# V2AI/EFG

Hardware: AMD Instinct MI355X
Metric: scenes/sec ConQueR 1-frame Waymo train step (higher is better)
Workload: dtype f32; 1 GPU; ConQueR res18 p3, 1-sweep Waymo-shaped scenes, 180000 pts/scene, 0.1 m voxels, 2 scenes/GPU, 900 queries, fwd+bwd+AdamW+OneCycle, graph of `value`: FPN levels / heads the reference evaluates and never reads are skipped (same losses and gradients; the line's `full_graph` object times the full reference graph); global_batch=2, parallelism=dp1

## Files before the change

efg_amd/_lib.py:

```python
import ctypes
import os

import torch

_LIB_PATH = os.path.join(os.path.dirname(os.path.abspath(__file__)), "lib", "libefg_hip.so")
_lib = None

c_void_p, c_int, c_int64, c_size_t, c_float = (ctypes.c_void_p, ctypes.c_int, ctypes.c_int64, ctypes.c_size_t,
                                               ctypes.c_float)

_SIGS = {
    "efg_last_error": (ctypes.c_char_p, []),
    "efg_version": (ctypes.c_char_p, []),
    "efg_capture_stream_create": (ctypes.c_int, [ctypes.POINTER(ctypes.c_void_p)]),
    "efg_capture_stream_destroy": (ctypes.c_int, [ctypes.c_void_p]),
    "efg_dynamic_voxelize_f32": (c_int, [c_void_p, c_int64, c_int, c_void_p, c_void_p, c_void_p, c_void_p]),
    "efg_hard_voxelize_workspace_bytes": (c_size_t, [c_int64, c_int, c_int, c_int, c_int, c_void_p, c_void_p]),
    "efg_hard_voxelize_f32": (c_int, [c_void_p, c_void_p, c_int, c_int, c_void_p, c_void_p, c_int, c_int, c_void_p,
                                      c_void_p, c_int, c_void_p, c_void_p, c_void_p, c_void_p, c_size_t, c_void_p]),
    "efg_hard_voxelize_debug_timeline": (c_size_t, [c_void_p]),
    "efg_scatter_workspace_bytes": (c_size_t, [c_int64, c_int, c_void_p]),
    "efg_scatter_index": (c_int, [c_void_p, c_int64, c_int, c_void_p, c_void_p, c_void_p, c_void_p, c_size_t,
                                  c_void_p]),
    "efg_scatter_reduce_workspace_bytes": (c_size_t, [c_int64, c_int]),
# ... 70 lines not shown
    "efg_focal_loss_forward_f32": (c_int, [c_void_p, c_void_p, c_int, c_int64, c_int, c_float, c_float, c_void_p, c_void_p,
                                           c_void_p]),
    "efg_focal_loss_backward_f32": (c_int, [c_void_p, c_void_p, c_int, c_int64, c_int, c_float, c_float, c_void_p,
                                            c_void_p, c_void_p, c_void_p]),
    "efg_box_loss_forward_f32": (c_int, [c_void_p] * 6 + [c_int64] + [c_int] * 4 + [c_void_p] * 3),
    "efg_box_loss_backward_f32": (c_int, [c_void_p] * 6 + [c_int64] + [c_int] * 4 + [c_void_p] * 4),
    "efg_rot_giou_paired_forward_f32": (c_int, [c_void_p, c_void_p, c_int64] + [c_void_p] * 4),
    "efg_rot_giou_paired_backward_f32": (c_int, [c_void_p, c_void_p, c_int64] + [c_void_p] * 5),
    "efg_match_cost_rot_f32": (c_int, [c_void_p] * 4 + [c_int] * 5 + [c_float] * 6 + [c_void_p] * 3),
    "efg_box_loss_rot_forward_f32": (c_int, [c_void_p] * 6 + [c_int64] + [c_int] * 4 + [c_void_p] * 4),
    "efg_box_loss_rot_backward_f32": (c_int, [c_void_p] * 6 + [c_int64] + [c_int] * 4 + [c_void_p] * 5),
    "efg_bn_workspace_bytes": (c_size_t, [c_int]),
    "efg_bn_forward_f32": (c_int, [c_void_p] * 7 + [c_float, c_float, c_int64, c_int, c_int] + [c_void_p] * 4 +
                           [c_size_t, c_void_p]),
    "efg_bn_backward_f32": (c_int, [c_void_p] * 6 + [c_int64, c_int, c_int] + [c_void_p] * 5 + [c_size_t, c_void_p]),
    "efg_lsap_f32": (c_int, [c_void_p, c_int, c_int, c_int, c_void_p, c_void_p, c_void_p, c_void_p]),
    "efg_nms_f32": (c_int, [c_void_p, c_int, c_float, c_int, c_void_p, c_void_p, c_void_p, c_size_t, c_void_p]),
    "efg_spconv_tile_shape": (c_int, [c_int, c_int, c_int, c_int64, c_int64, c_void_p, c_void_p, c_void_p]),
    "efg_cylinder_select_f32": (c_int, [c_void_p, c_int64, c_int, c_int, c_float, c_void_p, c_void_p, c_int64, c_void_p,
                                        c_void_p, c_void_p, c_int, c_void_p, c_void_p]),
    "efg_attention_fwd_f32": (c_int, [c_void_p, c_int64, c_int64, c_void_p, c_void_p, c_int64, c_int64, c_int64, c_int, c_int,
                                      c_int, c_float, c_void_p, c_void_p, c_void_p]),
    "efg_attention_bwd_f32": (c_int, [c_void_p, c_int64, c_int64, c_void_p, c_void_p, c_int64, c_int64, c_void_p, c_void_p,
                                      c_void_p, c_int64, c_int, c_int, c_int, c_float, c_void_p, c_void_p, c_void_p,
                                      c_void_p]),
    "efg_attention_long_fwd_f32": (c_int, [c_void_p, c_int64, c_int64] * 3 + [c_void_p, c_int, c_int64, c_int, c_int, c_float,
                                                                             c_void_p, c_void_p, c_void_p]),
    "efg_attention_long_bwd_f32": (c_int, [c_void_p, c_int64, c_int64] * 3 + [c_void_p, c_int, c_void_p, c_void_p, c_void_p,
                                                                             c_int64, c_int, c_int, c_float, c_void_p, c_void_p,
                                                                             c_void_p, c_void_p, c_void_p]),
# ... 107 lines not shown
```

efg_amd/csrc/batchnorm.hip:

```cpp
#include "common.h"

#include <algorithm>

namespace efg {
namespace {

constexpr int kBnBlocks = 1024;

__device__ __forceinline__ float4 ld4(const float* p) { return *reinterpret_cast<const float4*>(p); }
__device__ __forceinline__ void st4(float* p, float4 v) { *reinterpret_cast<float4*>(p) = v; }

struct Chunk {
  long long row_lo, row_hi;
};
__device__ __forceinline__ Chunk chunk_of(long long m, int nblocks, int b) {
  const long long per = (m + nblocks - 1) / nblocks;
  Chunk c;
  c.row_lo = min((long long)b * per, m);
  c.row_hi = min(c.row_lo + per, m);
  return c;
}

__device__ __forceinline__ float4 quad_sum(float4 v, int q4, float4* smem) {
  smem[threadIdx.x] = v;
// ... 206 lines not shown
    d.y = yy.y > 0.f ? d.y : 0.f;
    d.z = yy.z > 0.f ? d.z : 0.f;
    d.w = yy.w > 0.f ? d.w : 0.f;
  }
  if (dres) st4(dres + e * 4, d);
  const float4 mu = ld4(mean + ch), is = ld4(invstd + ch), ww = ld4(w + ch), a1 = ld4(dbias + ch), a2 = ld4(dweight + ch);
  const float inv_m = 1.0f / (float)m;
  float4 o;
  o.x = (d.x - a1.x * inv_m - (v.x - mu.x) * is.x * a2.x * inv_m) * is.x * ww.x;
  o.y = (d.y - a1.y * inv_m - (v.y - mu.y) * is.y * a2.y * inv_m) * is.y * ww.y;
  o.z = (d.z - a1.z * inv_m - (v.z - mu.z) * is.z * a2.z * inv_m) * is.z * ww.z;
  o.w = (d.w - a1.w * inv_m - (v.w - mu.w) * is.w * a2.w * inv_m) * is.w * ww.w;
  st4(dx + e * 4, o);
}


__global__ void __launch_bounds__(64)
gn_stats_merge_kernel(const float* __restrict__ partial, int nchunks, int c, int cpg, float eps,
                      float* __restrict__ mean_out, float* __restrict__ rstd_out) {
  const int lane = threadIdx.x, g = blockIdx.x, b = blockIdx.y, groups = c / cpg;
  const float* base = partial + (long long)b * nchunks * 3 * c;
  float cnt = 0.f, mean = 0.f, M2 = 0.f;
  const int items = nchunks * cpg;
  for (int i0 = lane; i0 < items; i0 += 64 * 8) {
    float nbv[8], mbv[8], qbv[8];
#pragma unroll
    for (int u = 0; u < 8; ++u) {
      const int i = min(i0 + 64 * u, items - 1);
      const float* p = base + (long long)(i / cpg) * 3 * c + g * cpg + i % cpg;
      nbv[u] = (i0 + 64 * u < items) ? p[0] : 0.f;
// ... 184 lines not shown
                "batch_norm backward: null pointer");
  EFG_CHECK_ARG(ws_bytes >= efg_bn_workspace_bytes(c), "batch_norm backward: workspace too small");
  hipStream_t st = (hipStream_t)stream;
  const int nb = nblocks_for(m);
  hipLaunchKernelGGL(bn_bwd_reduce_kernel, dim3(nb), dim3(256), 0, st, dy, x, y, mean, invstd, (long long)m, c, relu,
                     static_cast<float*>(ws));
  hipLaunchKernelGGL(bn_bwd_merge_kernel, dim3(2 * c), dim3(64), 0, st, static_cast<const float*>(ws), nb, c, dbias, dweight);
  EFG_LAUNCH_CHECK();
  const long long total4 = (long long)m * c / 4;
  hipLaunchKernelGGL(bn_bwd_apply_kernel, dim3((unsigned)ceil_div(total4, 256)), dim3(256), 0, st, dy, x, y, weight, mean,
                     invstd, dbias, dweight, total4, (long long)m, c, relu, dx, dresidual);
  EFG_LAUNCH_CHECK();
  return EFG_OK;
}

extern "C" size_t efg_gn_workspace_bytes(int batch, int c) {
  if (batch < 1 || c < 1) return 0;
  return align_up(sizeof(float) * ((size_t)batch * kBnBlocks * 3 * c + (size_t)batch * 4 * c), 256) + 256;
}

static int gn_check(int batch, int64_t rows, int c, int groups) {
  EFG_CHECK_ARG(batch >= 1 && batch <= 65535 && rows >= 1, "group_norm: need batch in [1, 65535] and rows >= 1");
  EFG_CHECK_ARG(c >= 4 && c % 4 == 0 && c <= 1024, "group_norm: need c %% 4 == 0 and c <= 1024 (got %d)", c);
  EFG_CHECK_ARG(groups >= 1 && c % groups == 0 && (c / groups) % 4 == 0,
                "group_norm: channels per group must be a multiple of 4 (c = %d, groups = %d)", c, groups);
  return EFG_OK;
}

extern "C" int efg_gn_forward_f32(const float* x, const float* weight, const float* bias, float eps, int batch,
                                  int64_t rows, int c, int groups, float* y, float* mean, float* rstd, void* ws,
// ... 40 lines not shown
```

efg_amd/modeling/backbones/fpn.py:

```python
import math

import torch.nn.functional as F
from torch import nn

from ..common import Conv2d, c2_xavier_fill, get_norm
from .sparse_net import ShapeSpec, _get, build_sparse_resnet_backbone


class LastLevelMaxPool(nn.Module):

    def __init__(self, in_feature="p5"):
        super().__init__()
        self.num_levels = 1
        self.in_feature = in_feature

    def forward(self, x):
        return [F.max_pool2d(x, kernel_size=1, stride=2, padding=0)]


class FPN(nn.Module):
    def __init__(self, bottom_up, in_features, out_channels, norm="", top_block=None, fuse_type="sum"):
        super().__init__()
        self.out_channels = out_channels
        input_shapes = bottom_up.output_shape()
# ... 35 lines not shown
    @property
    def size_divisibility(self):
        return self._size_divisibility

    def set_active_levels(self, levels):
        self.active_levels = None if levels is None else list(levels)
        if levels is None:
            self.bottom_up.dense_features = None
            return
        lvl_names = ["p{}".format(int(math.log2(s))) for s in
                     [self.bottom_up.output_shape()[f].stride for f in self.in_features]]
        need = [n in levels for n in lvl_names]
        first = min(i for i, n in enumerate(need) if n)
        self.bottom_up.dense_features = self.in_features[first:]

    def forward(self, *args, **kwargs):
        bottom_up_features = self.bottom_up(*args, **kwargs)
        self.__dict__["last_bottom_up"] = bottom_up_features
        levels = ["p{}".format(int(math.log2(self._out_feature_strides[n]))) for n in self._out_features]
        active = set(levels) if self.active_levels is None else set(self.active_levels)
        names_td = [n for n in self._out_features if n in
                    {"p{}".format(int(math.log2(self.bottom_up.output_shape()[f].stride))) for f in self.in_features}]
        names_td = names_td[::-1]
        feats = self.in_features[::-1]
        results = {}
        prev = None
        for name, f, lateral_conv, output_conv in zip(names_td, feats, self.lateral_convs, self.output_convs):
            finer_needed = any(n in active for n in names_td[names_td.index(name):])
            if not finer_needed:
                break
            lat = lateral_conv(bottom_up_features[f])
            if prev is not None:
                lat = lat + F.interpolate(prev, scale_factor=2, mode="nearest")
                if self._fuse_type == "avg":
                    lat = lat / 2
            prev = lat
            if name in active:
                results[name] = output_conv(prev)
        if self.top_block is not None:
            top_names = [n for n in self._out_features if n not in names_td]
            if any(n in active for n in top_names):
                src = bottom_up_features.get(self.top_block.in_feature, None)
                if src is None:
                    if self.top_block.in_feature not in results:
                        i = names_td.index(self.top_block.in_feature)
                        raise RuntimeError("top block input %s was not evaluated" % names_td[i])
                    src = results[self.top_block.in_feature]
                for n, r in zip(top_names, self.top_block(src)):
                    results[n] = r
        return {n: results[n] for n in self._out_features if n in results}

    def output_shape(self):
        return {name: ShapeSpec(channels=self._out_feature_channels[name], stride=self._out_feature_strides[name])
# ... 10 lines not shown
```

efg_amd/modeling/common/__init__.py:

```python
import os

import torch
import torch.nn.functional as F
from torch import nn

from ...operators import batchnorm as _bn
from ...operators import linear as _linear_mod
from ...operators.conv2d import arm_covers, conv3x3, conv3x3_arm, deterministic_mode
from ...operators.linear import linear


def get_norm(norm, out_channels):
    args = None
    if isinstance(norm, (list, tuple)):
        norm, args = norm
    if isinstance(norm, str):
        if len(norm) == 0:
            return None
        norm = {
            "BN": nn.BatchNorm2d,
            "BN1d": nn.BatchNorm1d,
            "GN": lambda channels: nn.GroupNorm(32, channels),
            "nnSyncBN": nn.SyncBatchNorm,
        }[norm]
# ... 7 lines not shown
    inplace = activation["inplace"] if isinstance(activation, dict) else activation.inplace
    return {"ReLU": nn.ReLU, "ReLU6": nn.ReLU6}[atype](inplace=inplace)


class Conv2d(nn.Conv2d):

    def __init__(self, *args, norm=None, activation=None, **kwargs):
        super().__init__(*args, **kwargs)
        self.norm = norm
        self.activation = activation

    def _is_pointwise(self):
        return (self.kernel_size == (1, 1) and self.stride == (1, 1) and self.padding == (0, 0)
                and self.dilation == (1, 1) and self.groups == 1)

    def forward(self, x):
        if self._is_pointwise():
            y = linear(x.permute(0, 2, 3, 1), self.weight.view(self.out_channels, self.in_channels), self.bias)
            x = y.permute(0, 3, 1, 2)
        elif (x.is_cuda and self.kernel_size == (3, 3) and self.stride == (1, 1) and self.padding == (1, 1)
              and self.dilation == (1, 1) and self.groups == 1 and torch.is_grad_enabled() and deterministic_mode()):
            x = conv3x3(x, self.weight, self.bias)
        elif (x.is_cuda and self.kernel_size == (3, 3) and self.stride == (1, 1) and self.padding == (1, 1)
              and self.dilation == (1, 1) and self.groups == 1 and torch.is_grad_enabled()
              and _linear_mod.arm_active() is not None
              and os.environ.get("EFG_CONV2D_ARM", "1") != "0" and arm_covers(x, self.weight)):
            x = conv3x3_arm(x, self.weight, self.bias)
        else:
            x = super().forward(x)
        if self.norm is not None:
            if _bn.fusable_nhwc(self.norm, x):
                relu = type(self.activation) is nn.ReLU
                x = _bn.bn_act_nhwc(x, self.norm, relu)
                if relu:
# ... 13 lines not shown
```

efg_amd/operators/batchnorm.py:

```python
import os

import torch
from torch.autograd import Function
from torch.autograd.function import once_differentiable

from .. import _lib as L

class BatchNormActFunction(Function):
    @staticmethod
    def forward(ctx, x, residual, weight, bias, running_mean, running_var, num_batches_tracked, momentum, eps, relu):
        x = x.contiguous()
        m, c = x.shape
        res = residual.contiguous() if residual is not None else None
        y = torch.empty_like(x)
        mean = torch.empty(c, dtype=torch.float32, device=x.device)
        invstd = torch.empty(c, dtype=torch.float32, device=x.device)
        ws_bytes = L.lib().efg_bn_workspace_bytes(c)
        ws = torch.empty(ws_bytes, dtype=torch.uint8, device=x.device)
        L.check(L.lib().efg_bn_forward_f32(L.ptr(x), L.ptr(res), L.ptr(weight), L.ptr(bias), L.ptr(running_mean),
                                           L.ptr(running_var), L.ptr(num_batches_tracked), float(momentum), float(eps),
                                           m, c, 1 if relu else 0, L.ptr(y), L.ptr(mean), L.ptr(invstd), L.ptr(ws),
                                           ws_bytes, L.stream()))
        ctx.save_for_backward(x, y, weight, mean, invstd)
        ctx.relu, ctx.has_residual = bool(relu), residual is not None
# ... 4 lines not shown
    @once_differentiable
    def backward(ctx, dy):
        x, y, weight, mean, invstd = ctx.saved_tensors
        m, c = x.shape
        dy = dy.contiguous()
        dx = torch.empty_like(x)
        dres = torch.empty_like(x) if ctx.has_residual else None
        dweight = torch.empty(c, dtype=torch.float32, device=x.device)
        dbias = torch.empty(c, dtype=torch.float32, device=x.device)
        ws_bytes = L.lib().efg_bn_workspace_bytes(c)
        ws = torch.empty(ws_bytes, dtype=torch.uint8, device=x.device)
        L.check(L.lib().efg_bn_backward_f32(L.ptr(dy), L.ptr(x), L.ptr(y), L.ptr(weight), L.ptr(mean), L.ptr(invstd), m,
                                            c, 1 if ctx.relu else 0, L.ptr(dx), L.ptr(dres), L.ptr(dweight),
                                            L.ptr(dbias), L.ptr(ws), ws_bytes, L.stream()))
        return dx, dres, dweight, dbias, None, None, None, None, None, None


def fusable(bn, x):
    return (os.environ.get("EFG_FUSED_BN", "1") != "0" and isinstance(bn, torch.nn.BatchNorm1d) and bn.training
            and bn.affine and bn.track_running_stats and bn.momentum is not None and x.is_cuda
            and x.dtype == torch.float32 and x.dim() == 2 and x.shape[0] >= 2 and x.shape[1] % 4 == 0
            and x.shape[1] <= 1024)


def bn_act(x, bn, relu=False, residual=None):
    if not fusable(bn, x):
        y = bn(x)
        if residual is not None:
            y = y + residual
        return torch.relu(y) if relu else y
# ... 33 lines not shown
```

efg_amd/operators/conv2d.py:

```python
import os

import torch
import torch.nn.functional as F
from torch.autograd import Function
from torch.autograd.function import once_differentiable

from .linear import arm_module, weight_grad


def deterministic_mode():
    return os.environ.get("EFG_DETERMINISTIC", "0") == "1"


def _pad_rows(t, front):
    b, c, h, w = t.shape
    r = b * (h + 2) * (w + 2)
    rows = (r + 15) // 16 * 16
    buf = torch.zeros((front + rows + front, c), dtype=t.dtype, device=t.device)
    buf[front:front + r].view(b, h + 2, w + 2, c)[:, 1:-1, 1:-1].copy_(t.permute(0, 2, 3, 1))
    return buf, r, rows


def _unpad_rows(flat, b, h, w):
    return flat[:b * (h + 2) * (w + 2)].view(b, h + 2, w + 2, -1)[:, 1:-1, 1:-1].permute(0, 3, 1, 2)


_TAPS = [(ky, kx) for ky in range(3) for kx in range(3)]


def _taps_gemm(buf, rows, front, wp, mats, sign, bias=None):
    out = (bias.expand(rows, -1).contiguous() if bias is not None else
           torch.zeros((rows, mats[0].shape[1]), dtype=buf.dtype, device=buf.device))
    for (ky, kx), m in zip(_TAPS, mats):
        s = front + sign * ((ky - 1) * wp + (kx - 1))
        out.addmm_(buf[s:s + rows], m)
    return out


def wgrad_3x3(x, gy, xb=None):
    b, ci, h, w = gy.shape[0], (x.shape[1] if xb is None else xb.shape[1]), gy.shape[2], gy.shape[3]
    co = gy.shape[1]
    wp = w + 2
    front = wp + 1
    if xb is None:
        xb, _, _ = _pad_rows(x, front)
    gb, _, rows = _pad_rows(gy, 0)
    parts = []
    for ky, kx in _TAPS:
        s = front + (ky - 1) * wp + (kx - 1)
        parts.append(weight_grad(xb[s:s + rows], gb))
    return torch.stack(parts, dim=-1).view(co, ci, 3, 3)


class Conv3x3Function(Function):
    @staticmethod
    def forward(ctx, x, weight, bias):
        b, _, h, w = x.shape
        front = w + 3
        xb, _, rows = _pad_rows(x, front)
        ctx.save_for_backward(xb, weight)
        ctx.has_bias = bias is not None
        ctx.geom = (b, h, w)
        mats = [weight[:, :, ky, kx].t() for ky, kx in _TAPS]
        return _unpad_rows(_taps_gemm(xb, rows, front, w + 2, mats, +1, bias), b, h, w)

    @staticmethod
    @once_differentiable
    def backward(ctx, gy):
        xb, weight = ctx.saved_tensors
        b, h, w = ctx.geom
        front = w + 3
        gx = gw = gb = None
        if ctx.needs_input_grad[0]:
            gbuf, _, rows = _pad_rows(gy, front)
            mats = [weight[:, :, ky, kx] for ky, kx in _TAPS]
            gx = _unpad_rows(_taps_gemm(gbuf, rows, front, w + 2, mats, -1), b, h, w)
        if ctx.needs_input_grad[1]:
            gw = wgrad_3x3(None, gy, xb=xb).contiguous(memory_format=torch.channels_last if weight.is_contiguous(
                memory_format=torch.channels_last) and not weight.is_contiguous() else torch.contiguous_format)
        if ctx.has_bias and ctx.needs_input_grad[2]:
            gb = gy.sum((0, 2, 3))
        return gx, gw, gb


def conv3x3(x, weight, bias):
    return Conv3x3Function.apply(x, weight, bias)


def _tap_rows(buf, start_row, rows, c):
    return buf.as_strided((rows, 3 * c), (c, 1), buf.storage_offset() + start_row * c)


def _arm_products():
    return arm_module(default="bf16x3")
# ... 61 lines not shown
```

include/efg_hip.h:

```cpp
#ifndef EFG_HIP_H
#define EFG_HIP_H
#include <stddef.h>
#include <stdint.h>

#ifdef __cplusplus
extern "C" {
#endif

#define EFG_OK 0
#define EFG_E_INVALID (-1)
#define EFG_E_WORKSPACE (-2)
#define EFG_E_HIP (-3)

const char* efg_last_error(void);
const char* efg_version(void);

int efg_capture_stream_create(void** stream_out);
int efg_capture_stream_destroy(void* stream);


int efg_dynamic_voxelize_f32(const float* points, int64_t n, int f, const float* voxel_size_host,
                             const float* coors_range_host, int32_t* coors, void* stream);

size_t efg_hard_voxelize_workspace_bytes(int64_t n_total, int batch, int f, int max_points, int max_voxels,
// ... 209 lines not shown
int efg_topk_unsorted_f32(const float* x, int64_t rows, int n, int k, float* values, int64_t* indices, void* stream);

int efg_box_refine_forward_f32(const float* delta, const float* anchor, int64_t n, float eps, float* out, void* stream);
int efg_box_refine_backward_f32(const float* grad, const float* out, const float* anchor, int64_t n, float eps,
                                float* grad_delta, float* grad_anchor, void* stream);

size_t efg_bn_workspace_bytes(int c);
int efg_bn_forward_f32(const float* x, const float* residual, const float* weight, const float* bias,
                       float* running_mean, float* running_var, int64_t* num_batches_tracked, float momentum, float eps,
                       int64_t m, int c, int relu, float* y, float* mean, float* invstd, void* ws, size_t ws_bytes,
                       void* stream);
int efg_bn_backward_f32(const float* dy, const float* x, const float* y, const float* weight, const float* mean,
                        const float* invstd, int64_t m, int c, int relu, float* dx, float* dresidual, float* dweight,
                        float* dbias, void* ws, size_t ws_bytes, void* stream);

size_t efg_gn_workspace_bytes(int batch, int c);
int efg_gn_forward_f32(const float* x, const float* weight, const float* bias, float eps, int batch, int64_t rows,
                       int c, int groups, float* y, float* mean, float* rstd, void* ws, size_t ws_bytes, void* stream);
int efg_gn_backward_f32(const float* dy, const float* x, const float* weight, const float* mean, const float* rstd,
                        int batch, int64_t rows, int c, int groups, float* dx, float* dweight, float* dbias, void* ws,
                        size_t ws_bytes, void* stream);

size_t efg_colsum_workspace_bytes(int64_t rows, int cols);
int efg_colsum_f32(const float* x, int64_t rows, int cols, int64_t row_stride, float* out, void* ws, size_t ws_bytes,
                   void* stream);
int efg_relu_bwd_colsum_f32(const float* g, const float* y, int64_t rows, int cols, float* g_out, float* out, void* ws,
                            size_t ws_bytes, void* stream);

size_t efg_gemm_bf16x3_pack_bytes(int k, int n);
int efg_gemm_bf16x3_pack_f32(const float* w, int64_t stride_k, int64_t stride_n, int k, int n, void* packed,
// ... 23 lines not shown
```

Baseline: 64.97 scenes/s.

## Run neck levels on padded NHWC row buffers with fused BN+upsample+pad kernels

Adds batch-norm kernels that read and write padded or compact row maps directly. The forward folds the nearest-2x upsampled coarse residual into the BN apply, and the backward folds the 2x2 pooling of the gradient into the dx pass. A new autograd function chains lateral BN, the 3x3 tap-GEMM conv and output BN on row buffers, so the separate pad/unpad copies, upsample-add and NCHW permutes per FPN level go away. It is enabled by default through an environment flag, at the cost of more kernel code and row-index arithmetic inside the kernels.

```diff
diff --git a/efg_amd/_lib.py b/efg_amd/_lib.py
--- a/efg_amd/_lib.py
+++ b/efg_amd/_lib.py
@@ -108,6 +108,12 @@
     "efg_bn_forward_f32": (c_int, [c_void_p] * 7 + [c_float, c_float, c_int64, c_int, c_int] + [c_void_p] * 4 +
                            [c_size_t, c_void_p]),
     "efg_bn_backward_f32": (c_int, [c_void_p] * 6 + [c_int64, c_int, c_int] + [c_void_p] * 5 + [c_size_t, c_void_p]),
+    "efg_bn_rows_workspace_bytes": (c_size_t, [c_int]),
+    "efg_bn_rows_padded_rows": (c_int64, [c_int, c_int, c_int, c_int64]),
+    "efg_bn_rows_forward_f32": (c_int, [c_void_p, c_int, c_int64] + [c_void_p] * 6 + [c_float, c_float] + [c_int] * 4 +
+                                [c_void_p, c_int, c_int64] + [c_void_p] * 3 + [c_size_t, c_void_p]),
+    "efg_bn_rows_backward_f32": (c_int, [c_void_p, c_int, c_int64] * 2 + [c_void_p] * 3 + [c_int] * 4 +
+                                 [c_void_p, c_int, c_int64] + [c_void_p] * 4 + [c_size_t, c_void_p]),
     "efg_lsap_f32": (c_int, [c_void_p, c_int, c_int, c_int, c_void_p, c_void_p, c_void_p, c_void_p]),
     "efg_nms_f32": (c_int, [c_void_p, c_int, c_float, c_int, c_void_p, c_void_p, c_void_p, c_size_t, c_void_p]),
     "efg_spconv_tile_shape": (c_int, [c_int, c_int, c_int, c_int64, c_int64, c_void_p, c_void_p, c_void_p]),
diff --git a/efg_amd/csrc/batchnorm.hip b/efg_amd/csrc/batchnorm.hip
--- a/efg_amd/csrc/batchnorm.hip
+++ b/efg_amd/csrc/batchnorm.hip
@@ -244,6 +244,252 @@
   st4(dx + e * 4, o);
 }
 
+struct RowMap {
+  int b, h, w, padded;
+  long long front;
+};
+struct RowPos {
+  int bi, y, x;
+};
+__device__ __forceinline__ long long phys_row(const RowMap& m, const RowPos& p) {
+  return m.padded ? m.front + ((long long)p.bi * (m.h + 2) + p.y + 1) * (m.w + 2) + p.x + 1
+                  : ((long long)p.bi * m.h + p.y) * m.w + p.x;
+}
+__device__ __forceinline__ RowPos pos_of(long long r, int h, int w) {
+  const long long plane = (long long)h * w;
+  long long bi = r / plane;
+  if (r - bi * plane < 0) --bi;
+  const int rem = (int)(r - bi * plane);
+  RowPos p;
+  p.bi = (int)bi;
+  p.y = rem / w;
+  p.x = rem % w;
+  return p;
+}
+__device__ __forceinline__ void advance(RowPos& p, int step, int h, int w) {
+  p.x += step;
+  if (p.x >= w) {
+    p.y += p.x / w;
+    p.x %= w;
+    if (p.y >= h) {
+      p.bi += p.y / h;
+      p.y %= h;
+    }
+  }
+}
+
+__global__ void __launch_bounds__(256)
+bn_stats_rows_kernel(const float* __restrict__ x, RowMap xm, int c, float* __restrict__ partial) {
+  __shared__ float4 smem[256];
+  const int q4 = c / 4, rstep = 256 / q4;
+  const int cq = threadIdx.x % q4, r0 = threadIdx.x / q4;
+  const bool lane_on = r0 < rstep;
+  const long long m = (long long)xm.b * xm.h * xm.w;
+  const Chunk ck = chunk_of(m, gridDim.x, blockIdx.x);
+  const float n = (float)(ck.row_hi - ck.row_lo);
+  float4 s = make_float4(0.f, 0.f, 0.f, 0.f);
+  if (lane_on) {
+    RowPos p = pos_of(ck.row_lo + r0, xm.h, xm.w);
+    for (long long r = ck.row_lo + r0; r < ck.row_hi; r += rstep) {
+      const float4 v = ld4(x + phys_row(xm, p) * c + cq * 4);
+      s.x += v.x;
+      s.y += v.y;
+      s.z += v.z;
+      s.w += v.w;
+      advance(p, rstep, xm.h, xm.w);
+    }
+  }
+  float4 tot = quad_sum(s, q4, smem);
+  if ((int)threadIdx.x < q4) smem[threadIdx.x] = make_float4(tot.x / fmaxf(n, 1.f), tot.y / fmaxf(n, 1.f), tot.z / fmaxf(n, 1.f), tot.w / fmaxf(n, 1.f));
+  __syncthreads();
+  const float4 mu = smem[cq];
+  __syncthreads();
+  float4 q = make_float4(0.f, 0.f, 0.f, 0.f);
+  if (lane_on) {
+    RowPos p = pos_of(ck.row_lo + r0, xm.h, xm.w);
+    for (long long r = ck.row_lo + r0; r < ck.row_hi; r += rstep) {
+      const float4 v = ld4(x + phys_row(xm, p) * c + cq * 4);
+      q.x += (v.x - mu.x) * (v.x - mu.x);
+      q.y += (v.y - mu.y) * (v.y - mu.y);
+      q.z += (v.z - mu.z) * (v.z - mu.z);
+      q.w += (v.w - mu.w) * (v.w - mu.w);
+      advance(p, rstep, xm.h, xm.w);
+    }
+  }
+  const float4 m2 = quad_sum(q, q4, smem);
+  if ((int)threadIdx.x < q4) {
+    float* pp = partial + (long long)blockIdx.x * 3 * c + cq * 4;
+    st4(pp, make_float4(n, n, n, n));
+    st4(pp + c, mu);
+    st4(pp + 2 * c, m2);
+  }
+}
+
+constexpr int kRowIters = 8;
+
+struct Drive {
+  int h, w, off;
+  long long shift, total;
+};
+__device__ __forceinline__ Drive drive_of(const RowMap& m, long long total) {
+  Drive d;
+  d.h = m.padded ? m.h + 2 : m.h;
+  d.w = m.padded ? m.w + 2 : m.w;
+  d.off = m.padded ? 1 : 0;
+  d.shift = m.padded ? m.front : 0;
+  d.total = total;
+  return d;
+}
+__device__ __forceinline__ bool image_pos(const Drive& dv, const RowMap& m, const RowPos& p, RowPos& img) {
+  img.bi = p.bi;
+  img.y = p.y - dv.off;
+  img.x = p.x - dv.off;
+  return p.bi >= 0 && p.bi < m.b && img.y >= 0 && img.y < m.h && img.x >= 0 && img.x < m.w;
+}
+
+__global__ void __launch_bounds__(256)
+bn_apply_rows_kernel(const float* __restrict__ x, RowMap xm, const float* __restrict__ coarse,
+                     const float* __restrict__ w, const float* __restrict__ b, const float* __restrict__ mean,
+                     const float* __restrict__ invstd, int c, float* __restrict__ y, RowMap ym, long long total) {
+  const int q4 = c / 4, rstep = 256 / q4;
+  const int cq = threadIdx.x % q4, r0 = threadIdx.x / q4;
+  if (r0 >= rstep) return;
+  const Drive dv = drive_of(ym, total);
+  long long d = (long long)blockIdx.x * rstep * kRowIters + r0;
+  RowPos p = pos_of(d - dv.shift, dv.h, dv.w);
+  const float4 mu = ld4(mean + cq * 4), is = ld4(invstd + cq * 4), ww = ld4(w + cq * 4), bb = ld4(b + cq * 4);
+#pragma unroll
+  for (int it = 0; it < kRowIters; ++it, d += rstep, advance(p, rstep, dv.h, dv.w)) {
+    if (d >= total) break;
+    RowPos img;
+    float4 o = make_float4(0.f, 0.f, 0.f, 0.f);
+    if (image_pos(dv, ym, p, img)) {
+      const float4 v = ld4(x + phys_row(xm, img) * c + cq * 4);
+      o.x = (v.x - mu.x) * is.x * ww.x + bb.x;
+      o.y = (v.y - mu.y) * is.y * ww.y + bb.y;
+      o.z = (v.z - mu.z) * is.z * ww.z + bb.z;
+      o.w = (v.w - mu.w) * is.w * ww.w + bb.w;
+      if (coarse) {
+        const long long rc = ((long long)img.bi * (ym.h / 2) + (img.y >> 1)) * (ym.w / 2) + (img.x >> 1);
+        const float4 r = ld4(coarse + rc * c + cq * 4);
+        o.x += r.x;
+        o.y += r.y;
+        o.z += r.z;
+        o.w += r.w;
+      }
+    }
+    st4(y + d * c + cq * 4, o);
+  }
+}
+
+__global__ void __launch_bounds__(256)
+bn_bwd_reduce_rows_kernel(const float* __restrict__ dy, RowMap dm, const float* __restrict__ x, RowMap xm,
+                          const float* __restrict__ mean, const float* __restrict__ invstd, int c,
+                          float* __restrict__ partial) {
+  __shared__ float4 smem[256];
+  const int q4 = c / 4, rstep = 256 / q4;
+  const int cq = threadIdx.x % q4, r0 = threadIdx.x / q4;
+  const bool lane_on = r0 < rstep;
+  const long long m = (long long)xm.b * xm.h * xm.w;
+  const Chunk ck = chunk_of(m, gridDim.x, blockIdx.x);
+  const float4 mu = ld4(mean + cq * 4), is = ld4(invstd + cq * 4);
+  float4 s1 = make_float4(0.f, 0.f, 0.f, 0.f), s2 = s1;
+  if (lane_on) {
+    RowPos p = pos_of(ck.row_lo + r0, xm.h, xm.w);
+    for (long long r = ck.row_lo + r0; r < ck.row_hi; r += rstep) {
+      const float4 d = ld4(dy + phys_row(dm, p) * c + cq * 4);
+      const float4 v = ld4(x + phys_row(xm, p) * c + cq * 4);
+      s1.x += d.x;
+      s1.y += d.y;
+      s1.z += d.z;
+      s1.w += d.w;
+      s2.x += d.x * (v.x - mu.x) * is.x;
+      s2.y += d.y * (v.y - mu.y) * is.y;
+      s2.z += d.z * (v.z - mu.z) * is.z;
+      s2.w += d.w * (v.w - mu.w) * is.w;
+      advance(p, rstep, xm.h, xm.w);
+    }
+  }
+  const float4 t1 = quad_sum(s1, q4, smem), t2 = quad_sum(s2, q4, smem);
+  if ((int)threadIdx.x < q4) {
+    float* pp = partial + (long long)blockIdx.x * 2 * c + cq * 4;
+    st4(pp, t1);
+    st4(pp + c, t2);
+  }
+}
+
+__device__ __forceinline__ float4 bn_dx(float4 d, float4 v, float4 mu, float4 is, float4 ww, float4 a1, float4 a2,
+                                        float inv_m) {
+  float4 o;
+  o.x = (d.x - a1.x * inv_m - (v.x - mu.x) * is.x * a2.x * inv_m) * is.x * ww.x;
+  o.y = (d.y - a1.y * inv_m - (v.y - mu.y) * is.y * a2.y * inv_m) * is.y * ww.y;
+  o.z = (d.z - a1.z * inv_m - (v.z - mu.z) * is.z * a2.z * inv_m) * is.z * ww.z;
+  o.w = (d.w - a1.w * inv_m - (v.w - mu.w) * is.w * a2.w * inv_m) * is.w * ww.w;
+  return o;
+}
+
+__global__ void __launch_bounds__(256)
+bn_bwd_apply_rows_kernel(const float* __restrict__ dy, RowMap dm, const float* __restrict__ x, RowMap xm,
+                         const float* __restrict__ w, const float* __restrict__ mean, const float* __restrict__ invstd,
+                         const float* __restrict__ dbias, const float* __restrict__ dweight, int c,
+                         float* __restrict__ dx, RowMap gm, long long total) {
+  const int q4 = c / 4, rstep = 256 / q4;
+  const int cq = threadIdx.x % q4, r0 = threadIdx.x / q4;
+  if (r0 >= rstep) return;
+  const Drive dv = drive_of(gm, total);
+  long long d = (long long)blockIdx.x * rstep * kRowIters + r0;
+  RowPos p = pos_of(d - dv.shift, dv.h, dv.w);
+  const float4 mu = ld4(mean + cq * 4), is = ld4(invstd + cq * 4), ww = ld4(w + cq * 4), a1 = ld4(dbias + cq * 4),
+               a2 = ld4(dweight + cq * 4);
+  const float inv_m = 1.0f / (float)((long long)gm.b * gm.h * gm.w);
+#pragma unroll
+  for (int it = 0; it < kRowIters; ++it, d += rstep, advance(p, rstep, dv.h, dv.w)) {
+    if (d >= total) break;
+    RowPos img;
+    float4 o = make_float4(0.f, 0.f, 0.f, 0.f);
+    if (image_pos(dv, gm, p, img))
+      o = bn_dx(ld4(dy + phys_row(dm, img) * c + cq * 4), ld4(x + phys_row(xm, img) * c + cq * 4), mu, is, ww, a1, a2,
+                inv_m);
+    st4(dx + d * c + cq * 4, o);
+  }
+}
+
+__global__ void __launch_bounds__(256)
+bn_bwd_apply_pool_kernel(const float* __restrict__ dy, RowMap dm, const float* __restrict__ x, RowMap xm,
+                         const float* __restrict__ w, const float* __restrict__ mean, const float* __restrict__ invstd,
+                         const float* __restrict__ dbias, const float* __restrict__ dweight, int c,
+                         float* __restrict__ dx, RowMap gm, float* __restrict__ dcoarse, long long total_coarse) {
+  const int q4 = c / 4, rstep = 256 / q4;
+  const int cq = threadIdx.x % q4, r0 = threadIdx.x / q4;
+  if (r0 >= rstep) return;
+  const int hc = gm.h / 2, wc = gm.w / 2;
+  long long rc = (long long)blockIdx.x * rstep * kRowIters + r0;
+  RowPos p = pos_of(rc, hc, wc);
+  const float4 mu = ld4(mean + cq * 4), is = ld4(invstd + cq * 4), ww = ld4(w + cq * 4), a1 = ld4(dbias + cq * 4),
+               a2 = ld4(dweight + cq * 4);
+  const float inv_m = 1.0f / (float)((long long)gm.b * gm.h * gm.w);
+#pragma unroll 2
+  for (int it = 0; it < kRowIters; ++it, rc += rstep, advance(p, rstep, hc, wc)) {
+    if (rc >= total_coarse) break;
+    float4 acc = make_float4(0.f, 0.f, 0.f, 0.f);
+#pragma unroll
+    for (int k = 0; k < 4; ++k) {
+      RowPos f;
+      f.bi = p.bi;
+      f.y = 2 * p.y + (k >> 1);
+      f.x = 2 * p.x + (k & 1);
+      const float4 d = ld4(dy + phys_row(dm, f) * c + cq * 4);
+      const float4 v = ld4(x + phys_row(xm, f) * c + cq * 4);
+      acc.x += d.x;
+      acc.y += d.y;
+      acc.z += d.z;
+      acc.w += d.w;
+      st4(dx + phys_row(gm, f) * c + cq * 4, bn_dx(d, v, mu, is, ww, a1, a2, inv_m));
+    }
+    st4(dcoarse + rc * c + cq * 4, acc);
+  }
+}
+
 
 __global__ void __launch_bounds__(64)
 gn_stats_merge_kernel(const float* __restrict__ partial, int nchunks, int c, int cpg, float eps,
@@ -458,6 +704,95 @@
   return EFG_OK;
 }
 
+extern "C" size_t efg_bn_rows_workspace_bytes(int c) { return efg_bn_workspace_bytes(c); }
+
+extern "C" int64_t efg_bn_rows_padded_rows(int b, int h, int w, int64_t front) {
+  if (b < 1 || h < 1 || w < 1 || front < 0) return 0;
+  const int64_t r = (int64_t)b * (h + 2) * (w + 2);
+  return front + (r + 15) / 16 * 16 + front;
+}
+
+static int bn_rows_check(const char* what, int b, int h, int w, int c, const int* padded, const int64_t* front, int nmaps) {
+  EFG_CHECK_ARG(c >= 4 && c % 4 == 0 && c <= 1024, "%s: need c %% 4 == 0 and c <= 1024 (got %d)", what, c);
+  EFG_CHECK_ARG(b >= 1 && h >= 1 && w >= 1, "%s: need b, h, w >= 1 (got %d, %d, %d)", what, b, h, w);
+  EFG_CHECK_ARG((int64_t)b * h * w >= 2, "%s: training statistics need at least two rows", what);
+  for (int i = 0; i < nmaps; ++i) {
+    EFG_CHECK_ARG(padded[i] == 0 || padded[i] == 1, "%s: padded is 0 or 1", what);
+    EFG_CHECK_ARG(front[i] >= 0 && (padded[i] || front[i] == 0), "%s: front >= 0, and 0 for a compact map", what);
+    EFG_CHECK_ARG(efg_bn_rows_padded_rows(b, h, w, front[i]) < (int64_t(1) << 31), "%s: map too large", what);
+  }
+  return EFG_OK;
+}
+
+static RowMap row_map(int b, int h, int w, int padded, int64_t front) {
+  RowMap m;
+  m.b = b, m.h = h, m.w = w, m.padded = padded, m.front = front;
+  return m;
+}
+static long long map_rows(const RowMap& m) {
+  return m.padded ? efg_bn_rows_padded_rows(m.b, m.h, m.w, m.front) : (long long)m.b * m.h * m.w;
+}
+static unsigned row_blocks(long long rows, int c) { return (unsigned)ceil_div(rows, (long long)(256 / (c / 4)) * kRowIters); }
+
+extern "C" int efg_bn_rows_forward_f32(const float* x, int x_padded, int64_t x_front, const float* coarse,
+                                       const float* weight, const float* bias, float* running_mean, float* running_var,
+                                       int64_t* num_batches_tracked, float momentum, float eps, int b, int h, int w,
+                                       int c, float* y, int y_padded, int64_t y_front, float* mean, float* invstd,
+                                       void* ws, size_t ws_bytes, void* stream) {
+  const int padded[2] = {x_padded, y_padded};
+  const int64_t front[2] = {x_front, y_front};
+  if (int rc = bn_rows_check("batch_norm rows", b, h, w, c, padded, front, 2)) return rc;
+  EFG_CHECK_ARG(x && weight && bias && y && mean && invstd && ws, "batch_norm rows: null pointer");
+  EFG_CHECK_ARG(!coarse || (h % 2 == 0 && w % 2 == 0), "batch_norm rows: the upsampled residual needs even h and w (got %d, %d)", h, w);
+  EFG_CHECK_ARG(ws_bytes >= efg_bn_workspace_bytes(c), "batch_norm rows: workspace too small");
+  EFG_CHECK_ARG((running_mean == nullptr) == (running_var == nullptr), "batch_norm rows: running_mean / running_var go together");
+  hipStream_t st = (hipStream_t)stream;
+  const RowMap xm = row_map(b, h, w, x_padded, x_front), ym = row_map(b, h, w, y_padded, y_front);
+  const int nb = nblocks_for((long long)b * h * w);
+  hipLaunchKernelGGL(bn_stats_rows_kernel, dim3(nb), dim3(256), 0, st, x, xm, c, static_cast<float*>(ws));
+  hipLaunchKernelGGL(bn_stats_merge_kernel, dim3(c), dim3(64), 0, st, static_cast<const float*>(ws), nb, c, eps, momentum,
+                     mean, invstd, running_mean, running_var, reinterpret_cast<long long*>(num_batches_tracked));
+  EFG_LAUNCH_CHECK();
+  const long long total = map_rows(ym);
+  hipLaunchKernelGGL(bn_apply_rows_kernel, dim3(row_blocks(total, c)), dim3(256), 0, st, x, xm, coarse, weight, bias, mean,
+                     invstd, c, y, ym, total);
+  EFG_LAUNCH_CHECK();
+  return EFG_OK;
+}
+
+extern "C" int efg_bn_rows_backward_f32(const float* dy, int dy_padded, int64_t dy_front, const float* x, int x_padded,
+                                        int64_t x_front, const float* weight, const float* mean, const float* invstd,
+                                        int b, int h, int w, int c, float* dx, int dx_padded, int64_t dx_front,
+                                        float* dcoarse, float* dweight, float* dbias, void* ws, size_t ws_bytes,
+                                        void* stream) {
+  const int padded[3] = {dy_padded, x_padded, dx_padded};
+  const int64_t front[3] = {dy_front, x_front, dx_front};
+  if (int rc = bn_rows_check("batch_norm rows backward", b, h, w, c, padded, front, 3)) return rc;
+  EFG_CHECK_ARG(dy && x && weight && mean && invstd && dx && dweight && dbias && ws, "batch_norm rows backward: null pointer");
+  EFG_CHECK_ARG(!dcoarse || (h % 2 == 0 && w % 2 == 0), "batch_norm rows backward: the pooled gradient needs even h and w (got %d, %d)", h, w);
+  EFG_CHECK_ARG(!dcoarse || !dx_padded, "batch_norm rows backward: the pooled gradient goes with a compact dx");
+  EFG_CHECK_ARG(ws_bytes >= efg_bn_workspace_bytes(c), "batch_norm rows backward: workspace too small");
+  hipStream_t st = (hipStream_t)stream;
+  const RowMap dm = row_map(b, h, w, dy_padded, dy_front), xm = row_map(b, h, w, x_padded, x_front),
+               gm = row_map(b, h, w, dx_padded, dx_front);
+  const int nb = nblocks_for((long long)b * h * w);
+  hipLaunchKernelGGL(bn_bwd_reduce_rows_kernel, dim3(nb), dim3(256), 0, st, dy, dm, x, xm, mean, invstd, c,
+                     static_cast<float*>(ws));
+  hipLaunchKernelGGL(bn_bwd_merge_kernel, dim3(2 * c), dim3(64), 0, st, static_cast<const float*>(ws), nb, c, dbias, dweight);
+  EFG_LAUNCH_CHECK();
+  if (dcoarse) {
+    const long long total = (long long)b * (h / 2) * (w / 2);
+    hipLaunchKernelGGL(bn_bwd_apply_pool_kernel, dim3(row_blocks(total, c)), dim3(256), 0, st, dy, dm, x, xm, weight, mean,
+                       invstd, dbias, dweight, c, dx, gm, dcoarse, total);
+  } else {
+    const long long total = map_rows(gm);
+    hipLaunchKernelGGL(bn_bwd_apply_rows_kernel, dim3(row_blocks(total, c)), dim3(256), 0, st, dy, dm, x, xm, weight, mean,
+                       invstd, dbias, dweight, c, dx, gm, total);
+  }
+  EFG_LAUNCH_CHECK();
+  return EFG_OK;
+}
+
 extern "C" size_t efg_gn_workspace_bytes(int batch, int c) {
   if (batch < 1 || c < 1) return 0;
   return align_up(sizeof(float) * ((size_t)batch * kBnBlocks * 3 * c + (size_t)batch * 4 * c), 256) + 256;
diff --git a/efg_amd/modeling/backbones/fpn.py b/efg_amd/modeling/backbones/fpn.py
--- a/efg_amd/modeling/backbones/fpn.py
+++ b/efg_amd/modeling/backbones/fpn.py
@@ -1,8 +1,12 @@
 import math
 
+import torch
 import torch.nn.functional as F
 from torch import nn
 
+from ...operators import batchnorm as _bn
+from ...operators import neck_rows as _neck
+from ...operators.conv2d import deterministic_mode
 from ..common import Conv2d, c2_xavier_fill, get_norm
 from .sparse_net import ShapeSpec, _get, build_sparse_resnet_backbone
 
@@ -73,6 +77,30 @@
         first = min(i for i, n in enumerate(need) if n)
         self.bottom_up.dense_features = self.in_features[first:]
 
+    def _level(self, lateral_conv, output_conv, x, prev, want_output, last):
+        fused = (_neck.enabled() and lateral_conv._is_pointwise() and lateral_conv.activation is None and x.is_cuda
+                 and x.dtype == torch.float32 and lateral_conv.norm is not None
+                 and (prev is None or self._fuse_type == "sum"))
+        if fused:
+            z = lateral_conv.pointwise(x)
+            fused = _bn.fusable_nhwc(lateral_conv.norm, z) and (prev is None or _neck.residual_fits(z, prev))
+            if (fused and want_output and last and deterministic_mode() and torch.is_grad_enabled()
+                    and output_conv._is_plain3x3() and output_conv.bias is None and output_conv.activation is None
+                    and output_conv.norm is not None and output_conv.out_channels == z.shape[1]
+                    and _bn.fusable_nhwc(output_conv.norm, z)):
+                return _neck.level_on_rows(z, prev, lateral_conv.norm, output_conv, output_conv.norm), None
+            if fused and prev is not None:
+                lat = _bn.bn_upsample_add_nhwc(z, prev, lateral_conv.norm)
+                return (output_conv(lat) if want_output else None), lat
+            lat = _bn.bn_act_nhwc(z, lateral_conv.norm) if fused else lateral_conv.norm(z)
+        else:
+            lat = lateral_conv(x)
+        if prev is not None:
+            lat = lat + F.interpolate(prev, scale_factor=2, mode="nearest")
+            if self._fuse_type == "avg":
+                lat = lat / 2
+        return (output_conv(lat) if want_output else None), lat
+
     def forward(self, *args, **kwargs):
         bottom_up_features = self.bottom_up(*args, **kwargs)
         self.__dict__["last_bottom_up"] = bottom_up_features
@@ -88,14 +116,10 @@
             finer_needed = any(n in active for n in names_td[names_td.index(name):])
             if not finer_needed:
                 break
-            lat = lateral_conv(bottom_up_features[f])
-            if prev is not None:
-                lat = lat + F.interpolate(prev, scale_factor=2, mode="nearest")
-                if self._fuse_type == "avg":
-                    lat = lat / 2
-            prev = lat
+            last = not any(n in active for n in names_td[names_td.index(name) + 1:])
+            out, prev = self._level(lateral_conv, output_conv, bottom_up_features[f], prev, name in active, last)
             if name in active:
-                results[name] = output_conv(prev)
+                results[name] = out
         if self.top_block is not None:
             top_names = [n for n in self._out_features if n not in names_td]
             if any(n in active for n in top_names):
diff --git a/efg_amd/modeling/common/__init__.py b/efg_amd/modeling/common/__init__.py
--- a/efg_amd/modeling/common/__init__.py
+++ b/efg_amd/modeling/common/__init__.py
@@ -45,10 +45,17 @@
         return (self.kernel_size == (1, 1) and self.stride == (1, 1) and self.padding == (0, 0)
                 and self.dilation == (1, 1) and self.groups == 1)
 
+    def _is_plain3x3(self):
+        return (self.kernel_size == (3, 3) and self.stride == (1, 1) and self.padding == (1, 1)
+                and self.dilation == (1, 1) and self.groups == 1 and self.padding_mode == "zeros")
+
+    def pointwise(self, x):
+        y = linear(x.permute(0, 2, 3, 1), self.weight.view(self.out_channels, self.in_channels), self.bias)
+        return y.permute(0, 3, 1, 2)
+
     def forward(self, x):
         if self._is_pointwise():
-            y = linear(x.permute(0, 2, 3, 1), self.weight.view(self.out_channels, self.in_channels), self.bias)
-            x = y.permute(0, 3, 1, 2)
+            x = self.pointwise(x)
         elif (x.is_cuda and self.kernel_size == (3, 3) and self.stride == (1, 1) and self.padding == (1, 1)
               and self.dilation == (1, 1) and self.groups == 1 and torch.is_grad_enabled() and deterministic_mode()):
             x = conv3x3(x, self.weight, self.bias)
diff --git a/efg_amd/operators/batchnorm.py b/efg_amd/operators/batchnorm.py
--- a/efg_amd/operators/batchnorm.py
+++ b/efg_amd/operators/batchnorm.py
@@ -42,6 +42,95 @@
                                             c, 1 if ctx.relu else 0, L.ptr(dx), L.ptr(dres), L.ptr(dweight),
                                             L.ptr(dbias), L.ptr(ws), ws_bytes, L.stream()))
         return dx, dres, dweight, dbias, None, None, None, None, None, None
+
+
+COMPACT = (0, 0)
+
+
+def map_rows(geom, rmap):
+    b, h, w = geom
+    return int(L.lib().efg_bn_rows_padded_rows(b, h, w, rmap[1])) if rmap[0] else b * h * w
+
+
+def _check_rows(t, geom, rmap, c, what):
+    assert t.is_cuda and t.dtype == torch.float32 and t.is_contiguous(), what + ": need contiguous fp32 device rows"
+    assert t.numel() == map_rows(geom, rmap) * c, "%s: %d elements for %d rows of %d" % (what, t.numel(), map_rows(geom, rmap), c)
+
+
+def bn_rows_forward(x, xmap, coarse, weight, bias, running_mean, running_var, num_batches_tracked, momentum, eps, geom,
+                    ymap, out=None):
+    b, h, w = geom
+    c = weight.shape[0]
+    _check_rows(x, geom, xmap, c, "bn_rows x")
+    if coarse is not None:
+        assert h % 2 == 0 and w % 2 == 0
+        _check_rows(coarse, (b, h // 2, w // 2), COMPACT, c, "bn_rows coarse")
+    y = out if out is not None else torch.empty((map_rows(geom, ymap), c), dtype=torch.float32, device=x.device)
+    _check_rows(y, geom, ymap, c, "bn_rows y")
+    mean = torch.empty(c, dtype=torch.float32, device=x.device)
+    invstd = torch.empty(c, dtype=torch.float32, device=x.device)
+    ws_bytes = L.lib().efg_bn_rows_workspace_bytes(c)
+    ws = torch.empty(ws_bytes, dtype=torch.uint8, device=x.device)
+    L.check(L.lib().efg_bn_rows_forward_f32(L.ptr(x), xmap[0], xmap[1], L.ptr(coarse), L.ptr(weight), L.ptr(bias),
+                                            L.ptr(running_mean), L.ptr(running_var), L.ptr(num_batches_tracked),
+                                            float(momentum), float(eps), b, h, w, c, L.ptr(y), ymap[0], ymap[1],
+                                            L.ptr(mean), L.ptr(invstd), L.ptr(ws), ws_bytes, L.stream()))
+    return y, mean, invstd
+
+
+def bn_rows_backward(dy, dmap, x, xmap, weight, mean, invstd, geom, gmap, pool, out=None):
+    b, h, w = geom
+    c = weight.shape[0]
+    _check_rows(dy, geom, dmap, c, "bn_rows dy")
+    _check_rows(x, geom, xmap, c, "bn_rows x")
+    dx = out if out is not None else torch.empty((map_rows(geom, gmap), c), dtype=torch.float32, device=x.device)
+    _check_rows(dx, geom, gmap, c, "bn_rows dx")
+    assert not pool or (h % 2 == 0 and w % 2 == 0 and not gmap[0])
+    dcoarse = torch.empty((b * (h // 2) * (w // 2), c), dtype=torch.float32, device=x.device) if pool else None
+    dweight = torch.empty(c, dtype=torch.float32, device=x.device)
+    dbias = torch.empty(c, dtype=torch.float32, device=x.device)
+    ws_bytes = L.lib().efg_bn_rows_workspace_bytes(c)
+    ws = torch.empty(ws_bytes, dtype=torch.uint8, device=x.device)
+    L.check(L.lib().efg_bn_rows_backward_f32(L.ptr(dy), dmap[0], dmap[1], L.ptr(x), xmap[0], xmap[1], L.ptr(weight),
+                                             L.ptr(mean), L.ptr(invstd), b, h, w, c, L.ptr(dx), gmap[0], gmap[1],
+                                             L.ptr(dcoarse), L.ptr(dweight), L.ptr(dbias), L.ptr(ws), ws_bytes,
+                                             L.stream()))
+    return dx, dcoarse, dweight, dbias
+
+
+def _nhwc_rows(t):
+    b, c, h, w = t.shape
+    return t.permute(0, 2, 3, 1).reshape(b * h * w, c)
+
+
+class BatchNormUpsampleAddFunction(Function):
+
+    @staticmethod
+    def forward(ctx, x, coarse, weight, bias, running_mean, running_var, num_batches_tracked, momentum, eps):
+        b, c, h, w = x.shape
+        xr, cr = _nhwc_rows(x).contiguous(), _nhwc_rows(coarse).contiguous()
+        y, mean, invstd = bn_rows_forward(xr, COMPACT, cr, weight, bias, running_mean, running_var, num_batches_tracked,
+                                          momentum, eps, (b, h, w), COMPACT)
+        ctx.save_for_backward(xr, weight, mean, invstd)
+        ctx.geom = (b, h, w)
+        ctx.mark_non_differentiable(*[t for t in (running_mean, running_var, num_batches_tracked) if t is not None])
+        return y.view(b, h, w, c).permute(0, 3, 1, 2)
+
+    @staticmethod
+    @once_differentiable
+    def backward(ctx, dy):
+        xr, weight, mean, invstd = ctx.saved_tensors
+        b, h, w = ctx.geom
+        c = weight.shape[0]
+        dx, dcoarse, dweight, dbias = bn_rows_backward(_nhwc_rows(dy).contiguous(), COMPACT, xr, COMPACT, weight, mean,
+                                                       invstd, ctx.geom, COMPACT, True)
+        return (dx.view(b, h, w, c).permute(0, 3, 1, 2), dcoarse.view(b, h // 2, w // 2, c).permute(0, 3, 1, 2), dweight,
+                dbias, None, None, None, None, None)
+
+
+def bn_upsample_add_nhwc(x, coarse, bn):
+    return BatchNormUpsampleAddFunction.apply(x, coarse, bn.weight, bn.bias, bn.running_mean, bn.running_var,
+                                              bn.num_batches_tracked, bn.momentum, bn.eps)
 
 
 def fusable(bn, x):
diff --git a/efg_amd/operators/conv2d.py b/efg_amd/operators/conv2d.py
--- a/efg_amd/operators/conv2d.py
+++ b/efg_amd/operators/conv2d.py
@@ -29,55 +29,96 @@
 
 
 def _taps_gemm(buf, rows, front, wp, mats, sign, bias=None):
-    out = (bias.expand(rows, -1).contiguous() if bias is not None else
-           torch.zeros((rows, mats[0].shape[1]), dtype=buf.dtype, device=buf.device))
-    for (ky, kx), m in zip(_TAPS, mats):
+    if bias is not None:
+        out = bias.expand(rows, -1).contiguous()
+    else:
+        out = torch.empty((rows, mats[0].shape[1]), dtype=buf.dtype, device=buf.device)
+    for k, ((ky, kx), m) in enumerate(zip(_TAPS, mats)):
         s = front + sign * ((ky - 1) * wp + (kx - 1))
-        out.addmm_(buf[s:s + rows], m)
+        if k == 0 and bias is None:
+            torch.mm(buf[s:s + rows], m, out=out)
+        else:
+            out.addmm_(buf[s:s + rows], m)
     return out
 
 
-def wgrad_3x3(x, gy, xb=None):
+def _tap_mats(weight, transposed):
+    if weight.is_contiguous():
+        w9 = (weight.permute(2, 3, 1, 0) if transposed else weight.permute(2, 3, 0, 1)).contiguous()
+        return [w9[ky, kx] for ky, kx in _TAPS]
+    return [weight[:, :, ky, kx].t() if transposed else weight[:, :, ky, kx] for ky, kx in _TAPS]
+
+
+def wgrad_3x3(x, gy, xb=None, gb=None):
     b, ci, h, w = gy.shape[0], (x.shape[1] if xb is None else xb.shape[1]), gy.shape[2], gy.shape[3]
     co = gy.shape[1]
     wp = w + 2
     front = wp + 1
     if xb is None:
         xb, _, _ = _pad_rows(x, front)
-    gb, _, rows = _pad_rows(gy, 0)
+    if gb is None:
+        gb, _, _ = _pad_rows(gy, 0)
+    return _wgrad_rows(xb, gb, w)
+
+
+def _wgrad_rows(xb, gb, w):
+    wp, front, rows = w + 2, w + 3, gb.shape[0]
     parts = []
     for ky, kx in _TAPS:
         s = front + (ky - 1) * wp + (kx - 1)
         parts.append(weight_grad(xb[s:s + rows], gb))
-    return torch.stack(parts, dim=-1).view(co, ci, 3, 3)
+    return torch.stack(parts, dim=-1).view(gb.shape[1], xb.shape[1], 3, 3)
+
+
+def padded_geometry(b, h, w):
+    front = w + 3
+    rows = (b * (h + 2) * (w + 2) + 15) // 16 * 16
+    return front, rows, front + rows + front
+
+
+def conv3x3_rows_forward(xb, weight, bias, geom):
+    b, h, w = geom
+    front, rows, total = padded_geometry(b, h, w)
+    assert xb.shape[0] == total and xb.is_contiguous()
+    return _taps_gemm(xb, rows, front, w + 2, _tap_mats(weight, True), +1, bias)
+
+
+def conv3x3_rows_backward(xb, gbuf, weight, geom, need_gx=True, need_gw=True):
+    b, h, w = geom
+    front, rows, total = padded_geometry(b, h, w)
+    assert gbuf.shape[0] == total and gbuf.is_contiguous()
+    gx = gw = None
+    if need_gx:
+        gx = _taps_gemm(gbuf, rows, front, w + 2, _tap_mats(weight, False), -1)
+    if need_gw:
+        gw = _wgrad_rows(xb, gbuf[front:front + rows], w).contiguous(
+            memory_format=torch.channels_last if weight.is_contiguous(memory_format=torch.channels_last)
+            and not weight.is_contiguous() else torch.contiguous_format)
+    return gx, gw
 
 
 class Conv3x3Function(Function):
+
     @staticmethod
     def forward(ctx, x, weight, bias):
         b, _, h, w = x.shape
-        front = w + 3
-        xb, _, rows = _pad_rows(x, front)
+        xb, _, _ = _pad_rows(x, w + 3)
         ctx.save_for_backward(xb, weight)
         ctx.has_bias = bias is not None
         ctx.geom = (b, h, w)
-        mats = [weight[:, :, ky, kx].t() for ky, kx in _TAPS]
-        return _unpad_rows(_taps_gemm(xb, rows, front, w + 2, mats, +1, bias), b, h, w)
+        return _unpad_rows(conv3x3_rows_forward(xb, weight, bias, ctx.geom), b, h, w)
 
     @staticmethod
     @once_differentiable
     def backward(ctx, gy):
         xb, weight = ctx.saved_tensors
         b, h, w = ctx.geom
-        front = w + 3
         gx = gw = gb = None
-        if ctx.needs_input_grad[0]:
-            gbuf, _, rows = _pad_rows(gy, front)
-            mats = [weight[:, :, ky, kx] for ky, kx in _TAPS]
-            gx = _unpad_rows(_taps_gemm(gbuf, rows, front, w + 2, mats, -1), b, h, w)
-        if ctx.needs_input_grad[1]:
-            gw = wgrad_3x3(None, gy, xb=xb).contiguous(memory_format=torch.channels_last if weight.is_contiguous(
-                memory_format=torch.channels_last) and not weight.is_contiguous() else torch.contiguous_format)
+        if ctx.needs_input_grad[0] or ctx.needs_input_grad[1]:
+            gbuf, _, _ = _pad_rows(gy, w + 3)
+            gx, gw = conv3x3_rows_backward(xb, gbuf, weight, ctx.geom, ctx.needs_input_grad[0], ctx.needs_input_grad[1])
+            if gx is not None:
+                gx = _unpad_rows(gx, b, h, w)
         if ctx.has_bias and ctx.needs_input_grad[2]:
             gb = gy.sum((0, 2, 3))
         return gx, gw, gb
diff --git a/efg_amd/operators/neck_rows.py b/efg_amd/operators/neck_rows.py
--- /dev/null
+++ b/efg_amd/operators/neck_rows.py
@@ -0,0 +1,59 @@
+import os
+
+import torch
+from torch.autograd import Function
+from torch.autograd.function import once_differentiable
+
+from . import batchnorm as _bn
+from .conv2d import conv3x3_rows_backward, conv3x3_rows_forward, padded_geometry
+
+
+def enabled():
+    return os.environ.get("EFG_NECK_ROWS", "1") != "0"
+
+
+class NeckLevelRowsFunction(Function):
+    @staticmethod
+    def forward(ctx, z, coarse, w1, b1, rm1, rv1, nbt1, mom1, eps1, conv_w, w2, b2, rm2, rv2, nbt2, mom2, eps2):
+        b, _, h, w = z.shape
+        geom = (b, h, w)
+        front = padded_geometry(b, h, w)[0]
+        zr = _bn._nhwc_rows(z).contiguous()
+        cr = _bn._nhwc_rows(coarse).contiguous() if coarse is not None else None
+        xb, mean1, invstd1 = _bn.bn_rows_forward(zr, _bn.COMPACT, cr, w1, b1, rm1, rv1, nbt1, mom1, eps1, geom, (1, front))
+        yb = conv3x3_rows_forward(xb, conv_w, None, geom)
+        y, mean2, invstd2 = _bn.bn_rows_forward(yb, (1, 0), None, w2, b2, rm2, rv2, nbt2, mom2, eps2, geom, _bn.COMPACT)
+        ctx.save_for_backward(zr, xb, yb, conv_w, w1, mean1, invstd1, w2, mean2, invstd2)
+        ctx.geom, ctx.has_coarse = geom, coarse is not None
+        ctx.mark_non_differentiable(*[t for t in (rm1, rv1, nbt1, rm2, rv2, nbt2) if t is not None])
+        return y.view(b, h, w, -1).permute(0, 3, 1, 2)
+
+    @staticmethod
+    @once_differentiable
+    def backward(ctx, dy):
+        zr, xb, yb, conv_w, w1, mean1, invstd1, w2, mean2, invstd2 = ctx.saved_tensors
+        b, h, w = geom = ctx.geom
+        front = padded_geometry(b, h, w)[0]
+        gbuf, _, dw2, db2 = _bn.bn_rows_backward(_bn._nhwc_rows(dy).contiguous(), _bn.COMPACT, yb, (1, 0), w2, mean2, invstd2,
+                                                 geom, (1, front), False)
+        gx, gw = conv3x3_rows_backward(xb, gbuf, conv_w, geom, True, ctx.needs_input_grad[9])
+        dz, dcoarse, dw1, db1 = _bn.bn_rows_backward(gx, (1, 0), zr, _bn.COMPACT, w1, mean1, invstd1, geom, _bn.COMPACT,
+                                                     ctx.has_coarse)
+        c = w1.shape[0]
+        dz = dz.view(b, h, w, c).permute(0, 3, 1, 2)
+        if dcoarse is not None:
+            dcoarse = dcoarse.view(b, h // 2, w // 2, c).permute(0, 3, 1, 2)
+        return (dz, dcoarse, dw1, db1, None, None, None, None, None, gw, dw2, db2, None, None, None, None, None)
+
+
+def _bn_args(bn):
+    return (bn.weight, bn.bias, bn.running_mean, bn.running_var, bn.num_batches_tracked, bn.momentum, bn.eps)
+
+
+def residual_fits(z, coarse):
+    return (z.shape[2] % 2 == 0 and z.shape[3] % 2 == 0 and coarse.is_cuda and coarse.dtype == torch.float32
+            and tuple(coarse.shape) == (z.shape[0], z.shape[1], z.shape[2] // 2, z.shape[3] // 2))
+
+
+def level_on_rows(z, coarse, lateral_bn, conv, output_bn):
+    return NeckLevelRowsFunction.apply(z, coarse, *_bn_args(lateral_bn), conv.weight, *_bn_args(output_bn))
diff --git a/include/efg_hip.h b/include/efg_hip.h
--- a/include/efg_hip.h
+++ b/include/efg_hip.h
@@ -247,6 +247,17 @@
                         const float* invstd, int64_t m, int c, int relu, float* dx, float* dresidual, float* dweight,
                         float* dbias, void* ws, size_t ws_bytes, void* stream);
 
+size_t efg_bn_rows_workspace_bytes(int c);
+int64_t efg_bn_rows_padded_rows(int b, int h, int w, int64_t front);
+int efg_bn_rows_forward_f32(const float* x, int x_padded, int64_t x_front, const float* coarse, const float* weight,
+                            const float* bias, float* running_mean, float* running_var, int64_t* num_batches_tracked,
+                            float momentum, float eps, int b, int h, int w, int c, float* y, int y_padded,
+                            int64_t y_front, float* mean, float* invstd, void* ws, size_t ws_bytes, void* stream);
+int efg_bn_rows_backward_f32(const float* dy, int dy_padded, int64_t dy_front, const float* x, int x_padded,
+                             int64_t x_front, const float* weight, const float* mean, const float* invstd, int b, int h,
+                             int w, int c, float* dx, int dx_padded, int64_t dx_front, float* dcoarse, float* dweight,
+                             float* dbias, void* ws, size_t ws_bytes, void* stream);
+
 size_t efg_gn_workspace_bytes(int batch, int c);
 int efg_gn_forward_f32(const float* x, const float* weight, const float* bias, float eps, int batch, int64_t rows,
                        int c, int groups, float* y, float* mean, float* rstd, void* ws, size_t ws_bytes, void* stream);
```

New measurement: 64.95 scenes/s. No clear change (-0.0%).
